# PJLab-ADG/DetZero

Hardware: AMD Instinct MI355X
Metric: LiDAR frames/sec (160k pts, 0.1m voxels) (higher is better)
Workload: dtype f32 as f16 pairs (hi+lo, 22-bit significand; 3 f16 MFMA per product, f32 accumulate)

## Files before the change

detzero_amd/csrc/head_cand.hip:

```cpp
#include "hgemm.h"

namespace dz {

constexpr int HC_C = 64;
constexpr int HC_CAND = 32;
constexpr int HC_THREADS = 192;
constexpr int HC_PIX_BYTES = HC_C * 4;
constexpr int HC_HROW = HC_PIX_BYTES + 16;
constexpr int HC_LDS_BYTES = 9 * HC_CAND * HC_HROW;
constexpr int HC_MAX_BRANCH = 4;

struct HcArgs {
    const unsigned char *shared;
    const unsigned long long *cand;
    const int *ncand;
    const unsigned char *w1, *w2;
    const float *s1, *b1, *s2, *b2;
    float *head;
    int h, w, k, cand_stride, w1_cout;
    int g_cout[HC_MAX_BRANCH], g_ooff[HC_MAX_BRANCH];
};

template <class M>
__global__ __launch_bounds__(HC_THREADS) __attribute__((amdgpu_waves_per_eu(2, 2))) void k_head_at_cand(HcArgs a) {
    extern __shared__ __attribute__((aligned(16))) unsigned char hid_s[];
    const int tid = threadIdx.x, lane = tid & 63, ty = tid >> 6;
    const int n = lane & 31, hh = lane >> 5;
    const int g = blockIdx.y, b = blockIdx.z;
    const int hw = a.h * a.w, hp = a.h + 2, wp = a.w + 2;
    const int ncand = min(min(a.ncand[b], a.k), a.cand_stride);
    const int slot = blockIdx.x * HC_CAND + n;
    if (blockIdx.x * HC_CAND >= ncand) return;
    const bool live = slot < ncand;
    int pix = 0, y = 0, x = 0;
    if (live) {
        const unsigned long long e = a.cand[(size_t)b * a.cand_stride + slot];
        const uint32_t flat = 0xFFFFFFFFu - (uint32_t)(e & 0xFFFFFFFFull);
        pix = (int)(flat % (uint32_t)hw);
        y = pix / a.w;
        x = pix - y * a.w;
    }
    const int hy = y + ty - 1;
    bool ok[3];
    const unsigned char *base[3];
#pragma unroll
    for (int tx = 0; tx < 3; ++tx) {
        const int hx = x + tx - 1;
        ok[tx] = live && hy >= 0 && hy < a.h && hx >= 0 && hx < a.w;
        base[tx] = a.shared + (ok[tx] ? (((size_t)b * hp + hy) * wp + hx) * HC_PIX_BYTES : (size_t)0);
    }
    f32x16 acc[2][3];
#pragma unroll
    for (int ct = 0; ct < 2; ++ct)
#pragma unroll
        for (int tx = 0; tx < 3; ++tx)
#pragma unroll
            for (int e = 0; e < 16; ++e) acc[ct][tx][e] = 0.f;
    const v4u zero4 = {0u, 0u, 0u, 0u};
    const unsigned char *const wrow = a.w1 + ((size_t)(g * HC_C + n) * HC_C) * 4;
    const size_t w_tap = (size_t)a.w1_cout * HC_C * 4, w_ct = (size_t)32 * HC_C * 4;
    for (int kc = 0; kc < HC_C / 32; ++kc) {
#pragma unroll
        for (int s = 0; s < 9; ++s) {
            const int ky = s / 3, kx = s - ky * 3;
            const size_t toff = (size_t)(ky * wp + kx) * HC_PIX_BYTES;
#pragma unroll
            for (int q = 0; q < 2; ++q) {
                const int koff = kc * 128 + q * 64 + hh * 32;
                v4u c_hi[2], c_lo[2], p_hi[3], p_lo[3];
#pragma unroll
                for (int ct = 0; ct < 2; ++ct) {
                    const unsigned char *wpn = wrow + s * w_tap + ct * w_ct + koff;
                    c_hi[ct] = *reinterpret_cast<const v4u *>(wpn);
                    c_lo[ct] = *reinterpret_cast<const v4u *>(wpn + 16);
                }
#pragma unroll
                for (int tx = 0; tx < 3; ++tx) {
                    p_hi[tx] = p_lo[tx] = zero4;
                    if (ok[tx]) {
                        const unsigned char *pp = base[tx] + toff + koff;
                        p_hi[tx] = *reinterpret_cast<const v4u *>(pp);
                        p_lo[tx] = *reinterpret_cast<const v4u *>(pp + 16);
                    }
                }
#pragma unroll
                for (int term = 3 - M::TERMS; term < 3; ++term)
#pragma unroll
                    for (int ct = 0; ct < 2; ++ct)
#pragma unroll
                        for (int tx = 0; tx < 3; ++tx)
                            acc[ct][tx] = M::mma(term == 0 ? c_lo[ct] : c_hi[ct], term == 1 ? p_lo[tx] : p_hi[tx], acc[ct][tx]);
            }
        }
    }
#pragma unroll
    for (int tx = 0; tx < 3; ++tx) {
        unsigned char *const row = hid_s + ((ty * 3 + tx) * HC_CAND + n) * HC_HROW;
#pragma unroll
        for (int ct = 0; ct < 2; ++ct) {
#pragma unroll
            for (int j = 0; j < 4; ++j) {
                const int ch = g * HC_C + ct * 32 + 8 * j + 4 * hh;
                float v[4];
#pragma unroll
                for (int e = 0; e < 4; ++e) v[e] = fmaxf(fmaf(acc[ct][tx][4 * j + e], a.s1[ch + e], a.b1[ch + e]), 0.f);
                uint2 hi, lo;
                split4<M>(v, hi, lo);
                if (!ok[tx]) hi = lo = make_uint2(0u, 0u);
                unsigned char *d = row + (ct * 4 + j) * 32 + hh * 8;
                *reinterpret_cast<uint2 *>(d) = hi;
                *reinterpret_cast<uint2 *>(d + 16) = lo;
            }
        }
    }
    __syncthreads();
    if (ty != 0) return;
    f32x16 out;
#pragma unroll
    for (int e = 0; e < 16; ++e) out[e] = 0.f;
    const unsigned char *const w2row = a.w2 + ((size_t)(g * 9 * 32 + n) * HC_C) * 4;
    for (int kc = 0; kc < HC_C / 32; ++kc) {
#pragma unroll
        for (int s = 0; s < 9; ++s) {
#pragma unroll
            for (int q = 0; q < 2; ++q) {
                const int koff = kc * 128 + q * 64 + hh * 32;
                const unsigned char *wpn = w2row + (size_t)s * 32 * HC_C * 4 + koff;
                const v4u c_hi = *reinterpret_cast<const v4u *>(wpn), c_lo = *reinterpret_cast<const v4u *>(wpn + 16);
                const unsigned char *pp = hid_s + (s * HC_CAND + n) * HC_HROW + koff;
                const v4u p_hi = *reinterpret_cast<const v4u *>(pp), p_lo = *reinterpret_cast<const v4u *>(pp + 16);
                if constexpr (M::TERMS == 3) {
                    out = M::mma(c_lo, p_hi, out);
                    out = M::mma(c_hi, p_lo, out);
                }
                out = M::mma(c_hi, p_hi, out);
            }
        }
    }
    if (live && hh == 0) {
        float *o = a.head + ((size_t)b * hw + pix) * 12 + a.g_ooff[g];
        const int gc = a.g_cout[g];
#pragma unroll
        for (int e = 0; e < 4; ++e) {
            if (e < gc) o[e] = fmaf(out[e], a.s2 ? a.s2[g * 32 + e] : 1.f, a.b2 ? a.b2[g * 32 + e] : 0.f);
        }
    }
}


constexpr int HF_CAND = 16;
constexpr int HF_HROW = HC_C + 4;

__global__ __launch_bounds__(HC_THREADS) void k_head_at_cand_f32(HcArgs a) {
    __shared__ __attribute__((aligned(16))) float hid_s[9 * HF_CAND * HF_HROW];
    __shared__ int pix_s[HF_CAND];
    __shared__ int ok_s[3][HF_CAND];
    const int tid = threadIdx.x, lane = tid & 63, ty = tid >> 6;
    const int r = lane & 15, g4 = lane >> 4;
    const int br = blockIdx.y, b = blockIdx.z;
    const int hw = a.h * a.w, hp = a.h + 2, wp = a.w + 2;
    const int ncand = min(min(a.ncand[b], a.k), a.cand_stride);
    if (blockIdx.x * HF_CAND >= ncand) return;
    const int slot = blockIdx.x * HF_CAND + r;
    const bool live = slot < ncand;
    int pix = 0, y = 0, x = 0;
    if (live) {
        const unsigned long long e = a.cand[(size_t)b * a.cand_stride + slot];
        const uint32_t flat = 0xFFFFFFFFu - (uint32_t)(e & 0xFFFFFFFFull);
        pix = (int)(flat % (uint32_t)hw);
        y = pix / a.w;
        x = pix - y * a.w;
    }
    const int hy = y + ty - 1;
    bool ok[3];
    const float *base[3];
    int okm = 0;
#pragma unroll
    for (int tx = 0; tx < 3; ++tx) {
        const int hx = x + tx - 1;
        ok[tx] = live && hy >= 0 && hy < a.h && hx >= 0 && hx < a.w;
        okm |= ok[tx] ? 1 << tx : 0;
        base[tx] = reinterpret_cast<const float *>(a.shared) + (ok[tx] ? (((size_t)b * hp + hy) * wp + hx) * HC_C : (size_t)0);
    }
    if (lane < HF_CAND) {
        ok_s[ty][lane] = okm;
        if (ty == 0) pix_s[lane] = live ? pix : -1;
    }
    __syncthreads();
    f32x4 acc[3][4];
#pragma unroll
    for (int tx = 0; tx < 3; ++tx)
#pragma unroll
        for (int nt = 0; nt < 4; ++nt) acc[tx][nt] = f32x4{0.f, 0.f, 0.f, 0.f};
    const float *const w1 = reinterpret_cast<const float *>(a.w1) + br * HC_C + r;
    for (int s = 0; s < 9; ++s) {
        const int ky = s / 3, kx = s - ky * 3;
        const size_t toff = (size_t)(ky * wp + kx) * HC_C;
#pragma unroll
        for (int kq = 0; kq < HC_C / 16; ++kq) {
            const int k0 = kq * 16 + g4 * 4;
            f32x4 av[3];
#pragma unroll
            for (int tx = 0; tx < 3; ++tx) {
                av[tx] = f32x4{0.f, 0.f, 0.f, 0.f};
                if (ok[tx]) av[tx] = *reinterpret_cast<const f32x4 *>(base[tx] + toff + k0);
            }
#pragma unroll
            for (int e = 0; e < 4; ++e) {
                float bv[4];
#pragma unroll
                for (int nt = 0; nt < 4; ++nt) bv[nt] = w1[((size_t)s * HC_C + k0 + e) * a.w1_cout + nt * 16];
#pragma unroll
                for (int tx = 0; tx < 3; ++tx)
#pragma unroll
                    for (int nt = 0; nt < 4; ++nt) acc[tx][nt] = __builtin_amdgcn_mfma_f32_16x16x4f32(av[tx][e], bv[nt], acc[tx][nt], 0, 0, 0);
            }
        }
    }
#pragma unroll
    for (int nt = 0; nt < 4; ++nt) {
        const int ch = br * HC_C + nt * 16 + r;
        const float sc = a.s1[ch], sh = a.b1[ch];
#pragma unroll
        for (int tx = 0; tx < 3; ++tx)
#pragma unroll
            for (int e = 0; e < 4; ++e) {
                const int c = 4 * g4 + e;
                const float v = fmaxf(fmaf(acc[tx][nt][e], sc, sh), 0.f);
                hid_s[((ty * 3 + tx) * HF_CAND + c) * HF_HROW + nt * 16 + r] = ((ok_s[ty][c] >> tx) & 1) ? v : 0.f;
            }
    }
    __syncthreads();
    if (ty != 0) return;
    f32x4 out = {0.f, 0.f, 0.f, 0.f};
    const float *const w2 = reinterpret_cast<const float *>(a.w2) + (size_t)br * 9 * HC_C * 16 + r;
    for (int s = 0; s < 9; ++s) {
#pragma unroll
        for (int kq = 0; kq < HC_C / 16; ++kq) {
            const int k0 = kq * 16 + g4 * 4;
            const f32x4 av = *reinterpret_cast<const f32x4 *>(hid_s + (s * HF_CAND + r) * HF_HROW + k0);
#pragma unroll
            for (int e = 0; e < 4; ++e) out = __builtin_amdgcn_mfma_f32_16x16x4f32(av[e], w2[((size_t)s * HC_C + k0 + e) * 16], out, 0, 0, 0);
        }
    }
    if (r < a.g_cout[br]) {
        const float sc = a.s2 ? a.s2[br * 16 + r] : 1.f, sh = a.b2 ? a.b2[br * 16 + r] : 0.f;
#pragma unroll
        for (int e = 0; e < 4; ++e) {
            const int px = pix_s[4 * g4 + e];
            if (px >= 0) a.head[((size_t)b * hw + px) * 12 + a.g_ooff[br] + r] = fmaf(out[e], sc, sh);
        }
    }
}

template <class M>
static int launch_head_at_cand(const HcArgs &a, int batch, int nbranch, hipStream_t stream) {
    static PerDeviceFlags lds_done;
    if (int rc_ = reserve_lds(reinterpret_cast<const void *>(&k_head_at_cand<M>), HC_LDS_BYTES, lds_done, "dz_head_at_candidates")) return rc_;
    hipLaunchKernelGGL((k_head_at_cand<M>), dim3(ceil_div(a.k, HC_CAND), nbranch, batch), dim3(HC_THREADS), HC_LDS_BYTES, stream, a);
    DZ_LAUNCH_CHECK();
    return DZ_OK;
}

}

using namespace dz;

extern "C" {

int dz_head_at_candidates_supported(int math, int channels) {
    return (math == DZ_MATH_F32 || math == DZ_MATH_F16X2 || math == DZ_MATH_BF16X2 || math == DZ_MATH_F16) && channels == HC_C ? 1 : 0;
}

int dz_head_at_candidates(const float *shared, int batch, int h, int w, const unsigned long long *cand, const int *d_ncand, int cand_stride,
                          int k, const float *w1, int w1_cout, const float *s1, const float *b1, const float *w2, const float *s2,
                          const float *b2, int nbranch, const int *h_g_cout, const int *h_g_ooff, float *head, int math, void *stream_) {
    hipStream_t stream = (hipStream_t)stream_;
    DZ_CHECK_ARG(dz_head_at_candidates_supported(math, HC_C), "dz_head_at_candidates: unknown math mode %d", math);
    DZ_CHECK_ARG(batch >= 0 && batch <= 65535 && h >= 1 && w >= 1 && k >= 1 && cand_stride >= k, "dz_head_at_candidates: bad sizes");
    DZ_CHECK_ARG(nbranch >= 1 && nbranch <= HC_MAX_BRANCH && w1_cout >= nbranch * HC_C && w1_cout % 32 == 0, "dz_head_at_candidates: bad branch layout");
    DZ_CHECK_ARG(shared && cand && d_ncand && w1 && s1 && b1 && w2 && head && h_g_cout && h_g_ooff, "dz_head_at_candidates: null pointer");
    if (batch == 0) return DZ_OK;
    HcArgs a{};
    for (int g = 0; g < nbranch; ++g) {
        DZ_CHECK_ARG(h_g_cout[g] >= 1 && h_g_cout[g] <= 4 && h_g_ooff[g] >= 0 && h_g_ooff[g] + h_g_cout[g] <= 12, "dz_head_at_candidates: bad columns of branch %d", g);
        a.g_cout[g] = h_g_cout[g];
        a.g_ooff[g] = h_g_ooff[g];
    }
    a.shared = reinterpret_cast<const unsigned char *>(shared);
    a.cand = cand; a.ncand = d_ncand;
    a.w1 = reinterpret_cast<const unsigned char *>(w1); a.w2 = reinterpret_cast<const unsigned char *>(w2);
    a.s1 = s1; a.b1 = b1; a.s2 = s2; a.b2 = b2; a.head = head;
    a.h = h; a.w = w; a.k = k; a.cand_stride = cand_stride; a.w1_cout = w1_cout;
    if (math == DZ_MATH_F32) {
        hipLaunchKernelGGL(k_head_at_cand_f32, dim3(ceil_div(k, HF_CAND), nbranch, batch), dim3(HC_THREADS), 0, stream, a);
        DZ_LAUNCH_CHECK();
        return DZ_OK;
    }
    if (math == DZ_MATH_F16X2) return launch_head_at_cand<MathF16>(a, batch, nbranch, stream);
    if (math == DZ_MATH_F16) return launch_head_at_cand<MathF16H>(a, batch, nbranch, stream);
    return launch_head_at_cand<MathBF16>(a, batch, nbranch, stream);
}

}
```

Before: 1147.

## Stage candidate pixels and conv weights through LDS with register prefetch pipeline

The candidate-head 3x3 conv previously had every lane read weights and neighbour pixels straight from global memory for each tap. It now loads them with coalesced buffer loads into registers one step ahead and stores them into padded LDS images. Each horizontal pixel strip is reused across the three kx taps, and MFMA operands are read from LDS. This trades redundant global traffic and latency for two block barriers per step and more register pressure. It also adds a 2 GiB size check required by the buffer resource.

```diff
diff --git a/detzero_amd/csrc/head_cand.hip b/detzero_amd/csrc/head_cand.hip
--- a/detzero_amd/csrc/head_cand.hip
+++ b/detzero_amd/csrc/head_cand.hip
@@ -9,6 +9,7 @@
 constexpr int HC_HROW = HC_PIX_BYTES + 16;
 constexpr int HC_LDS_BYTES = 9 * HC_CAND * HC_HROW;
 constexpr int HC_MAX_BRANCH = 4;
+constexpr int HC_STEPS = (HC_C / 32) * 9;
 
 struct HcArgs {
     const unsigned char *shared;
@@ -21,6 +22,26 @@
     int g_cout[HC_MAX_BRANCH], g_ooff[HC_MAX_BRANCH];
 };
 
+constexpr int HC_SROW = 128 + 16;
+constexpr int HC_PIX_IMG = 5 * HC_CAND * HC_SROW;
+constexpr int HC_W_IMG = 2 * 32 * HC_SROW;
+constexpr int HC_W_LOADS = (2 * 32 * 8 + HC_THREADS - 1) / HC_THREADS;
+static_assert(3 * HC_PIX_IMG + HC_W_IMG <= HC_LDS_BYTES, "the staging images must fit under the hidden rows");
+static_assert(2 * 32 * 8 > (HC_W_LOADS - 1) * HC_THREADS && 2 * 32 * 8 - (HC_W_LOADS - 1) * HC_THREADS == 128, "last weight piece: waves 0 and 1");
+
+__device__ __forceinline__ void hc_wave_sync() {
+    __builtin_amdgcn_fence(__ATOMIC_RELEASE, "wavefront");
+    __builtin_amdgcn_wave_barrier();
+    __builtin_amdgcn_fence(__ATOMIC_ACQUIRE, "wavefront");
+}
+
+__device__ __forceinline__ __amdgpu_buffer_rsrc_t hc_rsrc(const unsigned char *base, int bytes) {
+    return __builtin_amdgcn_make_buffer_rsrc(const_cast<unsigned char *>(base), 0, bytes, 0x00020000);
+}
+__device__ __forceinline__ v4u hc_load(__amdgpu_buffer_rsrc_t rsrc, uint32_t lane_off, int uniform_off) {
+    return __builtin_amdgcn_raw_buffer_load_b128(rsrc, (int)lane_off, uniform_off, 0);
+}
+
 template <class M>
 __global__ __launch_bounds__(HC_THREADS) __attribute__((amdgpu_waves_per_eu(2, 2))) void k_head_at_cand(HcArgs a) {
     extern __shared__ __attribute__((aligned(16))) unsigned char hid_s[];
@@ -29,26 +50,48 @@
     const int g = blockIdx.y, b = blockIdx.z;
     const int hw = a.h * a.w, hp = a.h + 2, wp = a.w + 2;
     const int ncand = min(min(a.ncand[b], a.k), a.cand_stride);
-    const int slot = blockIdx.x * HC_CAND + n;
     if (blockIdx.x * HC_CAND >= ncand) return;
-    const bool live = slot < ncand;
-    int pix = 0, y = 0, x = 0;
-    if (live) {
+    auto cell = [&](int c, int &pix, int &y, int &x) {
+        const int slot = blockIdx.x * HC_CAND + c;
+        pix = y = x = 0;
+        if (slot >= ncand) return false;
         const unsigned long long e = a.cand[(size_t)b * a.cand_stride + slot];
         const uint32_t flat = 0xFFFFFFFFu - (uint32_t)(e & 0xFFFFFFFFull);
         pix = (int)(flat % (uint32_t)hw);
         y = pix / a.w;
         x = pix - y * a.w;
-    }
-    const int hy = y + ty - 1;
+        return true;
+    };
+    int pix, y, x;
+    const bool live = cell(n, pix, y, x);
     bool ok[3];
-    const unsigned char *base[3];
 #pragma unroll
     for (int tx = 0; tx < 3; ++tx) {
-        const int hx = x + tx - 1;
+        const int hy = y + ty - 1, hx = x + tx - 1;
         ok[tx] = live && hy >= 0 && hy < a.h && hx >= 0 && hx < a.w;
-        base[tx] = a.shared + (ok[tx] ? (((size_t)b * hp + hy) * wp + hx) * HC_PIX_BYTES : (size_t)0);
-    }
+    }
+    const int sr = lane >> 3, sp = lane & 7;
+    const __amdgpu_buffer_rsrc_t prsrc = hc_rsrc(a.shared + (size_t)b * hp * wp * HC_PIX_BYTES, hp * wp * HC_PIX_BYTES);
+    uint32_t p0[4], p1[4], p4[4];
+#pragma unroll
+    for (int j = 0; j < 4; ++j) {
+        int pj, yj, xj;
+        const bool lj = cell(sr + 8 * j, pj, yj, xj);
+        const int hy = yj + ty - 1;
+        const bool rowok = lj && hy >= 0 && hy < a.h;
+        const uint32_t row = rowok ? (uint32_t)(hy * wp) : 0u;
+        p1[j] = (row + (rowok ? xj : 0)) * HC_PIX_BYTES + sp * 16;
+        p0[j] = (row + (rowok ? max(xj - 1, 0) : 0)) * HC_PIX_BYTES + sp * 16;
+        p4[j] = (row + (rowok ? min(xj + 3, wp - 1) : 0)) * HC_PIX_BYTES + sp * 16;
+    }
+    const int w_tap = a.w1_cout * HC_C * 4;
+    const __amdgpu_buffer_rsrc_t wrsrc = hc_rsrc(a.w1 + (size_t)g * HC_C * HC_C * 4, 9 * w_tap - g * HC_C * HC_C * 4);
+    const uint32_t woff = (tid >> 3) * HC_C * 4 + (tid & 7) * 16;
+    unsigned char *const pimg = hid_s + ty * HC_PIX_IMG, *const wimg = hid_s + 3 * HC_PIX_IMG;
+    unsigned char *const st_p = pimg + sr * HC_SROW + sp * 16;
+    unsigned char *const st_w = wimg + (tid >> 3) * HC_SROW + (tid & 7) * 16;
+    const unsigned char *const fr_p = pimg + n * HC_SROW + hh * 32;
+    const unsigned char *const fr_w = wimg + n * HC_SROW + hh * 32;
     f32x16 acc[2][3];
 #pragma unroll
     for (int ct = 0; ct < 2; ++ct)
@@ -56,43 +99,80 @@
         for (int tx = 0; tx < 3; ++tx)
 #pragma unroll
             for (int e = 0; e < 16; ++e) acc[ct][tx][e] = 0.f;
-    const v4u zero4 = {0u, 0u, 0u, 0u};
-    const unsigned char *const wrow = a.w1 + ((size_t)(g * HC_C + n) * HC_C) * 4;
-    const size_t w_tap = (size_t)a.w1_cout * HC_C * 4, w_ct = (size_t)32 * HC_C * 4;
-    for (int kc = 0; kc < HC_C / 32; ++kc) {
-#pragma unroll
-        for (int s = 0; s < 9; ++s) {
-            const int ky = s / 3, kx = s - ky * 3;
-            const size_t toff = (size_t)(ky * wp + kx) * HC_PIX_BYTES;
-#pragma unroll
-            for (int q = 0; q < 2; ++q) {
-                const int koff = kc * 128 + q * 64 + hh * 32;
-                v4u c_hi[2], c_lo[2], p_hi[3], p_lo[3];
-#pragma unroll
-                for (int ct = 0; ct < 2; ++ct) {
-                    const unsigned char *wpn = wrow + s * w_tap + ct * w_ct + koff;
-                    c_hi[ct] = *reinterpret_cast<const v4u *>(wpn);
-                    c_lo[ct] = *reinterpret_cast<const v4u *>(wpn + 16);
-                }
-#pragma unroll
-                for (int tx = 0; tx < 3; ++tx) {
-                    p_hi[tx] = p_lo[tx] = zero4;
-                    if (ok[tx]) {
-                        const unsigned char *pp = base[tx] + toff + koff;
-                        p_hi[tx] = *reinterpret_cast<const v4u *>(pp);
-                        p_lo[tx] = *reinterpret_cast<const v4u *>(pp + 16);
-                    }
-                }
-#pragma unroll
-                for (int term = 3 - M::TERMS; term < 3; ++term)
-#pragma unroll
-                    for (int ct = 0; ct < 2; ++ct)
-#pragma unroll
-                        for (int tx = 0; tx < 3; ++tx)
-                            acc[ct][tx] = M::mma(term == 0 ? c_lo[ct] : c_hi[ct], term == 1 ? p_lo[tx] : p_hi[tx], acc[ct][tx]);
-            }
-        }
-    }
+    v4u rp[3][4], rw[HC_W_LOADS];
+    auto fetch_w = [&](int d) {
+        const int kc = d / 9, s = d - kc * 9;
+#pragma unroll
+        for (int i = 0; i < HC_W_LOADS; ++i)
+            if (i + 1 < HC_W_LOADS || ty < 2) rw[i] = hc_load(wrsrc, woff, s * w_tap + kc * 128 + i * 24 * HC_C * 4);
+    };
+    auto refill = [](int d, int e, int &grp, int &c) {
+        const int G = d / 3, kx = d - G * 3;
+        grp = G; c = kx + 2;
+        if (e == 0) return true;
+        if (kx == 0) { c = e - 1; return d == 0; }
+        grp = G + 1; c = kx - 1;
+        return e == 1 && G + 1 < HC_STEPS / 3;
+    };
+    auto fetch_p = [&](int d) {
+#pragma unroll
+        for (int e = 0; e < 3; ++e) {
+            int grp = 0, c = 0;
+            if (!refill(d, e, grp, c)) continue;
+            const int kc = grp / 3, ky = grp - kc * 3;
+            const int prow = ky * wp * HC_PIX_BYTES + kc * 128;
+#pragma unroll
+            for (int j = 0; j < 4; ++j)
+                rp[e][j] = hc_load(prsrc, (c == 0 ? p0[j] : c == 4 ? p4[j] : p1[j]) + (c == 0 || c == 4 ? 0 : c - 1) * HC_PIX_BYTES, prow);
+        }
+    };
+    fetch_p(0);
+    fetch_w(0);
+#pragma unroll
+    for (int d = 0; d < HC_STEPS; ++d) {
+        const int kx = d % 3;
+        hc_wave_sync();
+#pragma unroll
+        for (int e = 0; e < 3; ++e) {
+            int grp = 0, c = 0;
+            if (!refill(d, e, grp, c)) continue;
+#pragma unroll
+            for (int j = 0; j < 4; ++j) *reinterpret_cast<v4u *>(st_p + (c * 32 + j * 8) * HC_SROW) = rp[e][j];
+        }
+        if (d > 0) __syncthreads();
+#pragma unroll
+        for (int i = 0; i < HC_W_LOADS; ++i)
+            if (i + 1 < HC_W_LOADS || ty < 2) *reinterpret_cast<v4u *>(st_w + i * 24 * HC_SROW) = rw[i];
+        __syncthreads();
+        if (d + 1 < HC_STEPS) {
+            fetch_p(d + 1);
+            fetch_w(d + 1);
+        }
+        __builtin_amdgcn_sched_barrier(0);
+#pragma unroll
+        for (int q = 0; q < 2; ++q) {
+            v4u c_hi[2], c_lo[2], p_hi[3], p_lo[3];
+#pragma unroll
+            for (int ct = 0; ct < 2; ++ct) {
+                c_hi[ct] = *reinterpret_cast<const v4u *>(fr_w + ct * 32 * HC_SROW + q * 64);
+                c_lo[ct] = *reinterpret_cast<const v4u *>(fr_w + ct * 32 * HC_SROW + q * 64 + 16);
+            }
+#pragma unroll
+            for (int tx = 0; tx < 3; ++tx) {
+                p_hi[tx] = *reinterpret_cast<const v4u *>(fr_p + (tx + kx) * 32 * HC_SROW + q * 64);
+                p_lo[tx] = *reinterpret_cast<const v4u *>(fr_p + (tx + kx) * 32 * HC_SROW + q * 64 + 16);
+            }
+#pragma unroll
+            for (int term = 3 - M::TERMS; term < 3; ++term)
+#pragma unroll
+                for (int ct = 0; ct < 2; ++ct)
+#pragma unroll
+                    for (int tx = 0; tx < 3; ++tx)
+                        acc[ct][tx] = M::mma(term == 0 ? c_lo[ct] : c_hi[ct], term == 1 ? p_lo[tx] : p_hi[tx], acc[ct][tx]);
+            __builtin_amdgcn_sched_barrier(0);
+        }
+    }
+    __syncthreads();
 #pragma unroll
     for (int tx = 0; tx < 3; ++tx) {
         unsigned char *const row = hid_s + ((ty * 3 + tx) * HC_CAND + n) * HC_HROW;
@@ -278,6 +358,7 @@
     hipStream_t stream = (hipStream_t)stream_;
     DZ_CHECK_ARG(dz_head_at_candidates_supported(math, HC_C), "dz_head_at_candidates: unknown math mode %d", math);
     DZ_CHECK_ARG(batch >= 0 && batch <= 65535 && h >= 1 && w >= 1 && k >= 1 && cand_stride >= k, "dz_head_at_candidates: bad sizes");
+    DZ_CHECK_ARG((long long)(h + 2) * (w + 2) * HC_PIX_BYTES < (1ll << 31) && w1_cout <= 65536, "dz_head_at_candidates: a frame of the shared map and the hidden weights must stay below 2 GiB");
     DZ_CHECK_ARG(nbranch >= 1 && nbranch <= HC_MAX_BRANCH && w1_cout >= nbranch * HC_C && w1_cout % 32 == 0, "dz_head_at_candidates: bad branch layout");
     DZ_CHECK_ARG(shared && cand && d_ncand && w1 && s1 && b1 && w2 && head && h_g_cout && h_g_ooff, "dz_head_at_candidates: null pointer");
     if (batch == 0) return DZ_OK;
```

New measurement: 1153 (median of 6 runs). Within noise of the previous version (+0.5%).
